# vlongle/pixie

Hardware: AMD Instinct MI355X
Metric: voxels/s (128^3 U-Net fwd) + MPM particle-steps/s (higher is better)
Workload: dtype f32 (operands split fp16 hi+lo, 3 f16 MFMAs/product, fp32 accumulate); 1 GPU; 128^3x64 feature grid -> SegmentationUNet+RegressionUNet forward (+argmax/one-hot combine), 1 scene per GPU per step; grid=128, feature_channels=64, parallelism=scene-parallel x1, executor=c+hip_graph

## Files before the change

pixie_amd/csrc/conv3d_f16x3.hip:

```cpp
#include <hip/hip_runtime.h>

#include <cstdlib>
#include <map>
#include <string>
#include <type_traits>

#include "../../include/pixie_hip.h"
#include "common.h"
#include "conv_plan.h"

namespace pixie {

typedef float f32x16 __attribute__((ext_vector_type(16)));
typedef _Float16 f16x8 __attribute__((ext_vector_type(8)));

constexpr int kW16HeaderU4 = 4;

struct Conv16Args {
    const float* in0; const float* in1;
    int c0, cin;
    int ID, IH, IW;
    int LD, LH, LW;
    int ups;
    int stride;
    int OD, OH, OW;
    const float* pro_a; const float* pro_b; const float* gamma; const float* beta;
    int act;
    const uint4* w16;
    const float* wf;
    const float* bias;
    int cout, coutp;
    const float* residual; float* out;
    const unsigned* amax0; const unsigned* amax1;
    float in_bound;
    int TX, TY, TZ, lTX, lTY;
    int tiles_x, tiles_y, tiles_z, n_tiles;
    int HX, HY, HZ, HYX, CS;
    unsigned mHX, mHYX;
    float* stats; unsigned* out_amax;
    float* partial; int chunks_per_slice;
    int epi_lds;
    const float* sk_in0; const float* sk_in1;
    int sk_c0, sk_cin;
    const uint4* sk_w16; const float* sk_bias;
    const unsigned* sk_amax0; const unsigned* sk_amax1;
};

__device__ __forceinline__ int fast_div16(int n, int d, unsigned magic) {
    return (d == 1) ? n : (int)__umulhi((unsigned)n, magic);
}
__device__ __forceinline__ float act16(float t, int act) {
    if (act == 1) return t > 0.0f ? t : 0.02f * t;
    if (act == 2) return t / (1.0f + __expf(-t));
    return t;
}
__device__ __forceinline__ float act16_staged(float t, int act) {
    if (act == 1) return fmaxf(t, 0.02f * t);
    if (act == 2) return t / (1.0f + __expf(-t));
    return t;
}
__device__ __forceinline__ int scale_exponent(float bound) {
    const unsigned bits = __float_as_uint(bound);
    const int eb = (int)((bits >> 23) & 0xffu) - 127;
    if (!(bound > 0.0f) || eb > 100) return 0;
    int e = 14 - eb;
    return e > 100 ? 100 : (e < -100 ? -100 : e);
}
__device__ __forceinline__ float pow2i(int e) { return __uint_as_float((unsigned)(e + 127) << 23); }

template <int KS, int MB, int NB, bool EX = false, bool SP = false, int SK = 0>
__device__ __forceinline__ void conv3d_f16x3_body(const Conv16Args& A) {
    static_assert(!SP || (KS == 3 && NB == 4 && !EX), "sub-pixel path: 3^3, two x parities x two voxel blocks per wave");
    static_assert(SK == 0 || (!EX && !SP), "folded skip (SK: 1 register-fed, 2 staged through LDS): f16x3, no sub-pixel form");
    extern __shared__ uint4 smem16[];
    constexpr int PAD = (KS == 3) ? 1 : 0;
    constexpr int NW = 4, NT = 64 * NW;
    const int bufsz = 4 * A.CS;

    const int tid = threadIdx.x;
    const int lane = tid & 63;
    const int wave = tid >> 6;
    const int kh = lane >> 5;
    const int l31 = lane & 31;

    int t = blockIdx.x;
    {
        const int per = (A.n_tiles + 7) >> 3;
        const int cand = (t & 7) * per + (t >> 3);
        if ((A.n_tiles & 7) == 0) t = cand;
    }
    int par = 0;
    if constexpr (SP) { par = t & 3; t >>= 2; }
    const int py = par & 1, pz = par >> 1;
    const int tx = t % A.tiles_x; t /= A.tiles_x;
    const int ty = t % A.tiles_y;
    const int tz = t / A.tiles_y;
    const int ox0 = tx * A.TX, oy0 = ty * A.TY, oz0 = tz * A.TZ;
    const int cout0 = blockIdx.y * (MB * 32);
    const int lx0 = SP ? ox0 - 1 : ox0 * A.stride - PAD;
    const int ly0 = SP ? oy0 - 1 + py : oy0 * A.stride - PAD;
    const int lz0 = SP ? oz0 - 1 + pz : oz0 * A.stride - PAD;
    const size_t ISP = (size_t)A.ID * A.IH * A.IW;
    const size_t OSP = (size_t)A.OD * A.OH * A.OW;

    int voff[NB];
    int ovox[NB];
    bool valid[NB];
#pragma unroll
    for (int nb = 0; nb < NB; ++nb) {
        if constexpr (SP) {
            const int px = nb >> 1;
            const int j = (wave * 2 + (nb & 1)) * 32 + l31;
            int x = j & (A.TX - 1);
            int y = (j >> A.lTX) & (A.TY - 1);
            int z = j >> (A.lTX + A.lTY);
            const int gx = 2 * (ox0 + x) + px, gy = 2 * (oy0 + y) + py, gz = 2 * (oz0 + z) + pz;
            const bool v = (z < A.TZ) && (gx < A.OW) && (gy < A.OH) && (gz < A.OD);
            if (!v) { x = 0; y = 0; z = 0; }
            voff[nb] = (z * A.HY + y) * A.HX + x + px + kh * A.CS;
            ovox[nb] = v ? (gz * A.OH + gy) * A.OW + gx : 0;
            valid[nb] = v;
            continue;
        }
        const int j = (wave * NB + nb) * 32 + l31;
        int x = j & (A.TX - 1);
        int y = (j >> A.lTX) & (A.TY - 1);
        int z = j >> (A.lTX + A.lTY);
        const bool v = (z < A.TZ) && (ox0 + x < A.OW) && (oy0 + y < A.OH) && (oz0 + z < A.OD);
        if (!v) { x = 0; y = 0; z = 0; }
        voff[nb] = ((z * A.HY + y) * A.HX + x) * A.stride + kh * A.CS;
        ovox[nb] = ((oz0 + z) * A.OH + (oy0 + y)) * A.OW + ox0 + x;
        valid[nb] = v;
    }

    float bound = A.in_bound;
    if (A.amax0) {
        bound = __uint_as_float(*A.amax0);
        if (A.amax1) bound = fmaxf(bound, __uint_as_float(*A.amax1));
    }
    const int ex = EX ? 0 : scale_exponent(bound);
    const float sx = pow2i(ex);

    f32x16 acc[MB][NB];
#pragma unroll
    for (int mb = 0; mb < MB; ++mb)
#pragma unroll
        for (int nb = 0; nb < NB; ++nb)
#pragma unroll
            for (int r = 0; r < 16; ++r) acc[mb][nb][r] = 0.0f;

    const int KG = A.cin >> 3;
    const size_t tap_stride = (size_t)KG * A.coutp;
    const size_t plane = (size_t)(SP ? 64 : KS * KS * KS) * tap_stride;
    const uint4* wHi = A.w16 + kW16HeaderU4 + (size_t)kh * A.coutp + cout0 + l31 + (size_t)(par * 16) * tap_stride;
    const uint4* wLo = wHi + plane;
    const float* wF = A.wf + (size_t)kh * A.coutp + cout0 + l31;

    constexpr int TAPS = KS * KS * KS;
    auto stage_chunk = [&](int c_base, uint4* buf, int stid, int nthr) {
        uint4* bHi = buf;
        uint4* bLo = buf + 2 * A.CS;
        float pa[16], pb[16];
        {
            float pv = 0.0f;
            if (A.pro_a) pv = (lane & 16) ? A.pro_b[c_base + (lane & 15)] : A.pro_a[c_base + (lane & 15)];
#pragma unroll
            for (int j = 0; j < 16; ++j) {
                pa[j] = __int_as_float(__builtin_amdgcn_readlane(__float_as_int(pv), j));
                pb[j] = __int_as_float(__builtin_amdgcn_readlane(__float_as_int(pv), 16 + j));
            }
        }
        const bool has_aff = A.gamma != nullptr;
        using T = std::true_type; using F = std::false_type;
        if constexpr (EX) {
            float* bF = reinterpret_cast<float*>(buf);
            for (int v0 = stid; v0 < A.CS; v0 += 2 * nthr) {
                float val[2][16];
                float gm[2], bt[2];
                int sidx[2];
                bool ok[2];
#pragma unroll
                for (int u = 0; u < 2; ++u) {
                    const int vox = v0 + u * nthr;
                    int rem = vox;
                    const int hz = fast_div16(rem, A.HYX, A.mHYX);
                    rem -= hz * A.HYX;
                    const int hy = fast_div16(rem, A.HX, A.mHX);
                    const int hx = rem - hy * A.HX;
                    const int lz = lz0 + hz, ly = ly0 + hy, lx = lx0 + hx;
                    ok[u] = vox < A.CS && (unsigned)lz < (unsigned)A.LD && (unsigned)ly < (unsigned)A.LH && (unsigned)lx < (unsigned)A.LW;
                    sidx[u] = ok[u] ? ((lz >> A.ups) * A.IH + (ly >> A.ups)) * A.IW + (lx >> A.ups) : 0;
                }
#pragma unroll
                for (int u = 0; u < 2; ++u) {
#pragma unroll
                    for (int j = 0; j < 16; ++j) {
                        const int cg = c_base + j;
                        const float* src = (cg < A.c0) ? (A.in0 + (size_t)cg * ISP) : (A.in1 + (size_t)(cg - A.c0) * ISP);
                        val[u][j] = src[sidx[u]];
                    }
                    gm[u] = 1.0f; bt[u] = 0.0f;
                    if (has_aff) { gm[u] = A.gamma[sidx[u]]; bt[u] = A.beta[sidx[u]]; }
                }
                auto convert = [&](auto has_pro, auto act_c) {
#pragma unroll
                    for (int u = 0; u < 2; ++u) {
                        const int vox = v0 + u * nthr;
#pragma unroll
                        for (int j = 0; j < 16; ++j) {
                            float t = val[u][j];
                            if (decltype(has_pro)::value) t = t * pa[j] + pb[j];
                            t = t * gm[u] + bt[u];
                            const float sc = ok[u] ? act16(t, decltype(act_c)::value) : 0.0f;
                            if (vox < A.CS) bF[j * A.CS + vox] = sc;
                        }
                    }
                };
                if (A.pro_a) {
                    if (A.act == 1) convert(T{}, std::integral_constant<int, 1>{});
                    else if (A.act == 2) convert(T{}, std::integral_constant<int, 2>{});
                    else convert(T{}, std::integral_constant<int, 0>{});
                } else {
                    if (A.act == 1) convert(F{}, std::integral_constant<int, 1>{});
                    else if (A.act == 2) convert(F{}, std::integral_constant<int, 2>{});
                    else convert(F{}, std::integral_constant<int, 0>{});
                }
            }
            return;
        }
        const int n_items = (A.CS + nthr - 1) / nthr;
        const float* gsrc = has_aff ? A.gamma : A.in0;
        const float* bsrc = has_aff ? A.beta : A.in0;
        constexpr bool BUF = KS == 3 && MB == 2 && NB >= 2 && !SP;
        const unsigned chb = 4u * (unsigned)ISP;
        const int j1 = A.c0 - c_base;
        const bool straddle = j1 > 0 && j1 < 16;
        const float* cbase = (j1 > 0) ? A.in0 + (size_t)c_base * ISP : A.in1 + (size_t)(c_base - A.c0) * ISP;
        const __amdgpu_buffer_rsrc_t rs = __builtin_amdgcn_make_buffer_rsrc(const_cast<float*>(cbase), 0, -1, 0x00020000);
        const __amdgpu_buffer_rsrc_t rsg = __builtin_amdgcn_make_buffer_rsrc(const_cast<float*>(gsrc), 0, -1, 0x00020000);
        const __amdgpu_buffer_rsrc_t rsb = __builtin_amdgcn_make_buffer_rsrc(const_cast<float*>(bsrc), 0, -1, 0x00020000);
        struct Item { float val[16]; float gm, bt; bool ok; };
        auto slot = [&](int vox, bool& ok) {
            int rem = vox;
            const int hz = fast_div16(rem, A.HYX, A.mHYX);
            rem -= hz * A.HYX;
            const int hy = fast_div16(rem, A.HX, A.mHX);
            const int hx = rem - hy * A.HX;
            const int lz = lz0 + hz, ly = ly0 + hy, lx = lx0 + hx;
            ok = vox < A.CS && (unsigned)lz < (unsigned)A.LD && (unsigned)ly < (unsigned)A.LH && (unsigned)lx < (unsigned)A.LW;
            return ok ? ((lz >> A.ups) * A.IH + (ly >> A.ups)) * A.IW + (lx >> A.ups) : 0;
        };
        auto load_with_pointers = [&](Item& it, int sidx) {
            it.gm = gsrc[sidx]; it.bt = bsrc[sidx];
#pragma unroll
            for (int j = 0; j < 16; ++j) {
                const int cg = c_base + j;
                const float* src = (cg < A.c0) ? (A.in0 + (size_t)cg * ISP) : (A.in1 + (size_t)(cg - A.c0) * ISP);
                it.val[j] = src[sidx];
            }
        };
        auto fetch = [&](Item& it, int vox) {
            const int sidx = slot(vox, it.ok);
            if constexpr (BUF) {
                const int voff = 4 * sidx;
                it.gm = __uint_as_float(__builtin_amdgcn_raw_buffer_load_b32(rsg, voff, 0, 0));
                it.bt = __uint_as_float(__builtin_amdgcn_raw_buffer_load_b32(rsb, voff, 0, 0));
#pragma unroll
                for (int j = 0; j < 16; ++j)
                    it.val[j] = __uint_as_float(__builtin_amdgcn_raw_buffer_load_b32(rs, voff, (int)((unsigned)j * chb), 0));
            } else {
                load_with_pointers(it, sidx);
            }
            __builtin_amdgcn_sched_barrier(0);
        };
        auto convert = [&](const Item& it, int vox, auto has_pro, auto act_c) {
            const float gm = has_aff ? it.gm : 1.0f, bt = has_aff ? it.bt : 0.0f;
            f16x8 vh[2], vl[2];
#pragma unroll
            for (int j = 0; j < 16; ++j) {
                float t = it.val[j];
                if (decltype(has_pro)::value) t = t * pa[j] + pb[j];
                t = t * gm + bt;
                const float sc = act16_staged(t, decltype(act_c)::value) * sx;
                const _Float16 h = (_Float16)sc;
                vh[j >> 3][j & 7] = h;
                vl[j >> 3][j & 7] = (_Float16)(sc - (float)h);
            }
            uint4 w[4] = {__builtin_bit_cast(uint4, vh[0]), __builtin_bit_cast(uint4, vh[1]), __builtin_bit_cast(uint4, vl[0]),
                          __builtin_bit_cast(uint4, vl[1])};
#pragma unroll
            for (int q = 0; q < 4; ++q) {
                w[q].x = it.ok ? w[q].x : 0u; w[q].y = it.ok ? w[q].y : 0u;
                w[q].z = it.ok ? w[q].z : 0u; w[q].w = it.ok ? w[q].w : 0u;
            }
            if (vox < A.CS) {
                bHi[vox] = w[0];
                bHi[A.CS + vox] = w[1];
                bLo[vox] = w[2];
                bLo[A.CS + vox] = w[3];
            }
            __builtin_amdgcn_sched_barrier(0);
        };
        auto pipeline = [&](auto has_pro, auto act_c) {
            Item a, b;
            int vox = stid;
            int left = n_items;
            if constexpr (BUF) {
                if (straddle) {
#pragma unroll 1
                    for (; left > 0; --left, vox += nthr) {
                        load_with_pointers(a, slot(vox, a.ok));
                        convert(a, vox, has_pro, act_c);
                    }
                    return;
                }
            }
            fetch(a, vox);
#pragma unroll 1
            for (; left > 2; left -= 2, vox += 2 * nthr) {
                fetch(b, vox + nthr);
                convert(a, vox, has_pro, act_c);
                fetch(a, vox + 2 * nthr);
                convert(b, vox + nthr, has_pro, act_c);
            }
            if (left == 2) {
                fetch(b, vox + nthr);
                convert(a, vox, has_pro, act_c);
                convert(b, vox + nthr, has_pro, act_c);
            } else {
                convert(a, vox, has_pro, act_c);
            }
        };
        if (A.pro_a) {
            if (A.act == 1) pipeline(T{}, std::integral_constant<int, 1>{});
            else if (A.act == 2) pipeline(T{}, std::integral_constant<int, 2>{});
            else pipeline(T{}, std::integral_constant<int, 0>{});
        } else {
            if (A.act == 1) pipeline(F{}, std::integral_constant<int, 1>{});
            else if (A.act == 2) pipeline(F{}, std::integral_constant<int, 2>{});
            else pipeline(F{}, std::integral_constant<int, 0>{});
        }
    };
    auto mfma_chunk = [&](int c_base, const uint4* buf) {
        __builtin_amdgcn_s_setprio(3);
        if constexpr (EX) {
            const float* ldsF = reinterpret_cast<const float*>(buf);
            const size_t tapw = (size_t)A.cin * A.coutp;
            const float* wc = wF + (size_t)c_base * A.coutp;
            float a[8][MB], an[8][MB];
#pragma unroll
            for (int kp = 0; kp < 8; ++kp)
#pragma unroll
                for (int mb = 0; mb < MB; ++mb) a[kp][mb] = wc[(size_t)(2 * kp) * A.coutp + mb * 32];
#pragma unroll 1
            for (int zy = 0; zy < KS * KS; ++zy) {
                const int dz = zy / KS, dy = zy - dz * KS;
                const int rowoff = (dz * A.HY + dy) * A.HX;
#pragma unroll
// ... 82 lines not shown
        f16x8 ah[MB], al[MB];
#pragma unroll
        for (int mb = 0; mb < MB; ++mb) {
            ah[mb] = __builtin_bit_cast(f16x8, wh[mb * 32]);
            al[mb] = __builtin_bit_cast(f16x8, wl[mb * 32]);
        }
#pragma unroll 1
        for (int zy = 0; zy < KS * KS; ++zy) {
            const int dz = zy / KS, dy = zy - dz * KS;
            const int rowoff = (dz * A.HY + dy) * A.HX;
#pragma unroll
            for (int dx = 0; dx < KS; ++dx) {
                const int tap = zy * KS + dx;
                const int nxt = (tap + 1 < TAPS) ? tap + 1 : tap;
                f16x8 ahn[MB], aln[MB];
#pragma unroll
                for (int mb = 0; mb < MB; ++mb) {
                    ahn[mb] = __builtin_bit_cast(f16x8, wh[(size_t)nxt * tap_stride + mb * 32]);
                    aln[mb] = __builtin_bit_cast(f16x8, wl[(size_t)nxt * tap_stride + mb * 32]);
                }
                __builtin_amdgcn_sched_barrier(0);
                f16x8 bh[NB], bl[NB];
#pragma unroll
                for (int nb = 0; nb < NB; ++nb) {
                    bh[nb] = __builtin_bit_cast(f16x8, ldsHi[voff[nb] + rowoff + dx]);
                    bl[nb] = __builtin_bit_cast(f16x8, ldsLo[voff[nb] + rowoff + dx]);
                }
#pragma unroll
                for (int mb = 0; mb < MB; ++mb)
#pragma unroll
                    for (int nb = 0; nb < NB; ++nb)
                        acc[mb][nb] = __builtin_amdgcn_mfma_f32_32x32x16_f16(al[mb], bh[nb], acc[mb][nb], 0, 0, 0);
#pragma unroll
                for (int mb = 0; mb < MB; ++mb)
#pragma unroll
                    for (int nb = 0; nb < NB; ++nb)
                        acc[mb][nb] = __builtin_amdgcn_mfma_f32_32x32x16_f16(ah[mb], bl[nb], acc[mb][nb], 0, 0, 0);
#pragma unroll
                for (int mb = 0; mb < MB; ++mb)
#pragma unroll
                    for (int nb = 0; nb < NB; ++nb)
                        acc[mb][nb] = __builtin_amdgcn_mfma_f32_32x32x16_f16(ah[mb], bh[nb], acc[mb][nb], 0, 0, 0);
#pragma unroll
                for (int mb = 0; mb < MB; ++mb) { ah[mb] = ahn[mb]; al[mb] = aln[mb]; }
            }
        }
        __builtin_amdgcn_s_setprio(0);
    };

    float inv2 = 0.0f;
    {
        const int c_begin = A.partial ? (int)blockIdx.z * A.chunks_per_slice * 16 : 0;
        const int c_end = A.partial ? min(A.cin, c_begin + A.chunks_per_slice * 16) : A.cin;
        for (int c_base = c_begin; c_base < c_end; c_base += 16) {
            __syncthreads();
            stage_chunk(c_base, smem16, tid, NT);
            __syncthreads();
            mfma_chunk(c_base, smem16);
        }
        if constexpr (SK != 0) {
            float sb = __uint_as_float(*A.sk_amax0);
            if (A.sk_amax1) sb = fmaxf(sb, __uint_as_float(*A.sk_amax1));
            const int ex2 = scale_exponent(sb);
            const float sx2 = pow2i(ex2);
            const float inv_main = __uint_as_float(A.w16[0].x) * pow2i(-ex);
            inv2 = __uint_as_float(A.sk_w16[0].x) * pow2i(-ex2);
            const float ratio = inv_main / inv2;
#pragma unroll
            for (int mb = 0; mb < MB; ++mb)
#pragma unroll
                for (int nb = 0; nb < NB; ++nb)
#pragma unroll
                    for (int r = 0; r < 16; ++r) acc[mb][nb][r] *= ratio;
            auto sk_chunks = [&]() {
                int l31s = l31, khs = kh, waves = wave;
                asm volatile("" : "+v"(l31s), "+v"(khs), "+v"(waves));
                const unsigned chb = 4u * (unsigned)ISP;
                unsigned off[NB];
#pragma unroll
                for (int nb = 0; nb < NB; ++nb) {
                    const int j = (waves * NB + nb) * 32 + l31s;
                    const int x = j & (A.TX - 1), y = (j >> A.lTX) & (A.TY - 1), z = j >> (A.lTX + A.lTY);
                    off[nb] = (valid[nb] ? 4u * (unsigned)(((oz0 + z) * A.IH + (oy0 + y)) * A.IW + ox0 + x) : 0u) + 8u * (unsigned)khs * chb;
                }
                const unsigned wlane = 16u * (unsigned)(khs * A.coutp + l31s);
                const char* w2Hi = reinterpret_cast<const char*>(A.sk_w16 + kW16HeaderU4 + cout0);
                const char* w2Lo = w2Hi + (size_t)(A.sk_cin >> 3) * A.coutp * sizeof(uint4);
#pragma unroll 1
                for (int c2 = 0; c2 < A.sk_cin; c2 += 16) {
                    f16x8 ah[MB], al[MB];
                    const size_t wrow = (size_t)(c2 >> 3) * A.coutp * sizeof(uint4);
#pragma unroll
                    for (int mb = 0; mb < MB; ++mb) {
                        al[mb] = __builtin_bit_cast(f16x8, *reinterpret_cast<const uint4*>(w2Lo + wrow + mb * 32 * sizeof(uint4) + wlane));
                        ah[mb] = __builtin_bit_cast(f16x8, *reinterpret_cast<const uint4*>(w2Hi + wrow + mb * 32 * sizeof(uint4) + wlane));
                    }
                    const float* base = (c2 < A.sk_c0) ? (A.sk_in0 + (size_t)c2 * ISP) : (A.sk_in1 + (size_t)(c2 - A.sk_c0) * ISP);
                    const __amdgpu_buffer_rsrc_t rsrc = __builtin_amdgcn_make_buffer_rsrc(const_cast<float*>(base), 0, -1, 0x00020000);
                    float v[NB][8];
#pragma unroll
                    for (int q = 0; q < 8; ++q)
#pragma unroll
                        for (int nb = 0; nb < NB; ++nb)
                            v[nb][q] = __uint_as_float(__builtin_amdgcn_raw_buffer_load_b32(rsrc, (int)off[nb], (int)((unsigned)q * chb), 0));
                    __builtin_amdgcn_sched_barrier(0);
                    f16x8 bh[NB], bl[NB];
#pragma unroll
                    for (int nb = 0; nb < NB; ++nb)
#pragma unroll
                        for (int q = 0; q < 8; ++q) {
                            const float sc = valid[nb] ? v[nb][q] * sx2 : 0.0f;
// ... 55 lines not shown
                            vl[q >> 3][q & 7] = (_Float16)(sc - (float)hq);
                        }
                        const int slot = (z * A.HY + y) * A.HX + x + centre;
                        bHi[slot] = __builtin_bit_cast(uint4, vh[0]);
                        bHi[A.CS + slot] = __builtin_bit_cast(uint4, vh[1]);
                        bLo[slot] = __builtin_bit_cast(uint4, vl[0]);
                        bLo[A.CS + slot] = __builtin_bit_cast(uint4, vl[1]);
                    }
                    __syncthreads();
                    f16x8 bh[NB], bl[NB];
#pragma unroll
                    for (int nb = 0; nb < NB; ++nb) {
                        bh[nb] = __builtin_bit_cast(f16x8, bHi[voff[nb] + centre]);
                        bl[nb] = __builtin_bit_cast(f16x8, bLo[voff[nb] + centre]);
                    }
#pragma unroll
                    for (int mb = 0; mb < MB; ++mb)
#pragma unroll
                        for (int nb = 0; nb < NB; ++nb)
                            acc[mb][nb] = __builtin_amdgcn_mfma_f32_32x32x16_f16(al[mb], bh[nb], acc[mb][nb], 0, 0, 0);
#pragma unroll
                    for (int mb = 0; mb < MB; ++mb)
#pragma unroll
                        for (int nb = 0; nb < NB; ++nb)
                            acc[mb][nb] = __builtin_amdgcn_mfma_f32_32x32x16_f16(ah[mb], bl[nb], acc[mb][nb], 0, 0, 0);
#pragma unroll
                    for (int mb = 0; mb < MB; ++mb)
#pragma unroll
                        for (int nb = 0; nb < NB; ++nb)
                            acc[mb][nb] = __builtin_amdgcn_mfma_f32_32x32x16_f16(ah[mb], bh[nb], acc[mb][nb], 0, 0, 0);
                }
            } else {
                sk_chunks();
            }
        }
    }

    const float inv = EX ? 1.0f : (SK != 0 ? inv2 : __uint_as_float(A.w16[0].x) * pow2i(-ex));
    if (A.partial) {
        float* dst = A.partial + (size_t)blockIdx.z * A.cout * OSP;
#pragma unroll
        for (int mb = 0; mb < MB; ++mb)
#pragma unroll
            for (int r = 0; r < 16; ++r) {
                const int co = cout0 + mb * 32 + (r & 3) + 8 * (r >> 2) + 4 * kh;
                if (co < A.cout) {
#pragma unroll
                    for (int nb = 0; nb < NB; ++nb)
                        if (valid[nb]) dst[(size_t)co * OSP + ovox[nb]] = acc[mb][nb][r] * inv;
                }
            }
        return;
    }
    float* red = reinterpret_cast<float*>(smem16);
    float wmax = 0.0f;
    const bool full = SP ? (A.epi_lds && cout0 + MB * 32 <= A.cout && (A.TX & 1) == 0 && (A.OW & 3) == 0 && NW * 64 <= A.TX * A.TY * A.TZ &&
                            2 * (ox0 + A.TX) <= A.OW && 2 * (oy0 + A.TY) <= A.OH && 2 * (oz0 + A.TZ) <= A.OD)
                         : (A.epi_lds && cout0 + MB * 32 <= A.cout && (A.TX & 3) == 0 && (A.OW & 3) == 0 && NW * NB * 32 <= A.TX * A.TY * A.TZ &&
                            ox0 + A.TX <= A.OW && oy0 + A.TY <= A.OH && oz0 + A.TZ <= A.OD);
    if (full) {
        constexpr int LDO = NB * 32 + 4;
        float* ldsO = reinterpret_cast<float*>(smem16) + wave * (32 * LDO);
        red = reinterpret_cast<float*>(smem16) + NW * 32 * LDO;
        constexpr int LPR = NB * 8;
        constexpr int RPI = 32 / LPR;
        constexpr int NIT = 16 / RPI;
        constexpr int G = 4;
        constexpr int GPB = NIT / G;
        constexpr int NGRP = MB * GPB;
        const int rsub = l31 / LPR, colq = 4 * (l31 % LPR), nbq = colq >> 5;
        const float* nobias = EX ? A.wf : reinterpret_cast<const float*>(A.w16);
        const bool hb0 = A.bias != nullptr, hb1 = A.sk_bias != nullptr;
        float braw[MB][2];
#pragma unroll
        for (int mb = 0; mb < MB; ++mb) {
            braw[mb][0] = (hb0 ? A.bias : nobias)[cout0 + mb * 32 + l31];
            braw[mb][1] = (hb1 ? A.sk_bias : nobias)[cout0 + mb * 32 + l31];
        }
        __syncthreads();
        const int jq = SP ? wave * 64 + (colq >> 1) : (wave * NB + nbq) * 32 + (colq & 31);
        const int xq = jq & (A.TX - 1), yq = (jq >> A.lTX) & (A.TY - 1), zq = jq >> (A.lTX + A.lTY);
        const size_t ovq = SP ? ((size_t)(2 * (oz0 + zq) + pz) * A.OH + (2 * (oy0 + yq) + py)) * A.OW + 2 * (ox0 + xq)
                              : ((size_t)(oz0 + zq) * A.OH + (oy0 + yq)) * A.OW + ox0 + xq;
        const size_t orow0 = (size_t)(cout0 + kh * RPI + rsub) * OSP + ovq;
        auto rows = [&](auto res_c, auto stats_c) {
            constexpr bool RES = decltype(res_c)::value, STATS = decltype(stats_c)::value;
            size_t step = (size_t)(2 * RPI) * OSP;
            asm volatile("" : "+s"(step));
            const float* pr = A.residual + orow0;
            float* po = A.out + orow0;
            float4 r4[2][G];
            auto fetch = [&](int q) {
#pragma unroll
                for (int g = 0; g < G; ++g) { r4[q & 1][g] = *reinterpret_cast<const float4*>(pr); pr += step; }
            };
#pragma unroll
            for (int q = 0; q < NGRP; ++q) {
                const int mb = q / GPB, it0 = (q % GPB) * G;
                asm volatile("" ::: "memory");
                if (q % GPB == 0) {
                    const int brow = __float_as_int((hb0 ? braw[mb][0] : 0.0f) + (hb1 ? braw[mb][1] : 0.0f));
#pragma unroll
                    for (int r = 0; r < 16; ++r) {
                        const int row = (r & 3) + 8 * (r >> 2);
                        const int blo = __builtin_amdgcn_readlane(brow, row), bhi = __builtin_amdgcn_readlane(brow, row + 4);
                        const float bv = __int_as_float(kh ? bhi : blo);
#pragma unroll
                        for (int nb = 0; nb < NB; ++nb)
                            ldsO[((r & 3) + 8 * (r >> 2) + 4 * kh) * LDO + (SP ? 2 * ((nb & 1) * 32 + l31) + (nb >> 1) : nb * 32 + l31)] =
                                __builtin_fmaf(acc[mb][nb][r], inv, bv);
                    }
                }
                if constexpr (RES) {
                    if (q == 0) fetch(0);
                    if (q + 1 < NGRP) fetch(q + 1);
                }
                float4 v4[G];
#pragma unroll
                for (int g = 0; g < G; ++g) {
                    const int rowl = (2 * (it0 + g) + kh) * RPI + rsub;
                    v4[g] = *reinterpret_cast<const float4*>(ldsO + rowl * LDO + colq);
                    if constexpr (RES) { v4[g].x += r4[q & 1][g].x; v4[g].y += r4[q & 1][g].y; v4[g].z += r4[q & 1][g].z; v4[g].w += r4[q & 1][g].w; }
                    *reinterpret_cast<float4*>(po) = v4[g]; po += step;
                }
                if constexpr (STATS) {
                    float s1[G], s2[G];
#pragma unroll
                    for (int g = 0; g < G; ++g) {
                        const float4 v = v4[g];
                        s1[g] = (v.x + v.y) + (v.z + v.w);
                        s2[g] = (v.x * v.x + v.y * v.y) + (v.z * v.z + v.w * v.w);
                        wmax = fmaxf(fmaxf(wmax, fmaxf(fabsf(v.x), fabsf(v.y))), fmaxf(fabsf(v.z), fabsf(v.w)));
                    }
                    asm volatile("" : "+v"(wmax));
#pragma unroll
                    for (int off = LPR / 2; off > 0; off >>= 1) {
                        float t1[G], t2[G];
#pragma unroll
                        for (int g = 0; g < G; ++g) { t1[g] = __shfl_xor(s1[g], off, 64); t2[g] = __shfl_xor(s2[g], off, 64); }
#pragma unroll
                        for (int g = 0; g < G; ++g) { s1[g] += t1[g]; s2[g] += t2[g]; }
                    }
                    if ((l31 % LPR) == 0) {
#pragma unroll
                        for (int g = 0; g < G; ++g) {
                            const int rowl = (2 * (it0 + g) + kh) * RPI + rsub;
                            red[(wave * MB * 32 + mb * 32 + rowl) * 2] = s1[g]; red[(wave * MB * 32 + mb * 32 + rowl) * 2 + 1] = s2[g];
                        }
                    }
                }
            }
        };
        using T = std::true_type; using F = std::false_type;
        if (A.residual) { if (A.stats) rows(T{}, T{}); else rows(T{}, F{}); }
        else { if (A.stats) rows(F{}, T{}); else rows(F{}, F{}); }
    } else {
    if (A.stats) __syncthreads();
#pragma unroll
    for (int mb = 0; mb < MB; ++mb) {
#pragma unroll
        for (int r = 0; r < 16; ++r) {
            const int row = mb * 32 + (r & 3) + 8 * (r >> 2) + 4 * kh;
            const int co = cout0 + row;
            float s1 = 0.0f, s2 = 0.0f;
            if (co < A.cout) {
                const float bv = (A.bias ? A.bias[co] : 0.0f) + (A.sk_bias ? A.sk_bias[co] : 0.0f);
#pragma unroll
                for (int nb = 0; nb < NB; ++nb) {
                    if (valid[nb]) {
                        const size_t o = (size_t)co * OSP + ovox[nb];
                        float val = acc[mb][nb][r] * inv + bv;
                        if (A.residual) val += A.residual[o];
                        A.out[o] = val;
                        s1 += val; s2 += val * val; wmax = fmaxf(wmax, fabsf(val));
                    }
                }
            }
            if (A.stats) {
#pragma unroll
                for (int off = 16; off > 0; off >>= 1) { s1 += __shfl_xor(s1, off, 64); s2 += __shfl_xor(s2, off, 64); }
                if (l31 == 0) { red[(wave * MB * 32 + row) * 2] = s1; red[(wave * MB * 32 + row) * 2 + 1] = s2; }
            }
        }
    }
    }
    if (A.stats) {
        __syncthreads();
        if (tid < MB * 32 * 2) {
            float t = red[tid];
#pragma unroll
            for (int w = 1; w < NW; ++w) t += red[w * MB * 64 + tid];
            A.stats[((size_t)blockIdx.x * A.coutp + cout0) * 2 + tid] = t;
        }
        if (A.out_amax) {
#pragma unroll
            for (int off = 32; off > 0; off >>= 1) wmax = fmaxf(wmax, __shfl_xor(wmax, off, 64));
            if (lane == 0 && wmax > 0.0f) atomicMax(A.out_amax, __float_as_uint(wmax));
        }
    }
}

template <int KS, int MB, int NB>
__global__ __launch_bounds__(256, 2) void conv3d_f16x3_kernel(Conv16Args A) {
    conv3d_f16x3_body<KS, MB, NB>(A);
}
template <int KS, int MB, int NB, bool STAGED>
__global__ __launch_bounds__(256, 2) void conv3d_f16x3_skip_kernel(Conv16Args A) {
    conv3d_f16x3_body<KS, MB, NB, false, false, STAGED ? 2 : 1>(A);
}
template <int KS, int MB, int NB>
__global__ __launch_bounds__(256, 2) void conv3d_exact_kernel(Conv16Args A) {
    conv3d_f16x3_body<KS, MB, NB, true>(A);
}
template <int MB>
__global__ __launch_bounds__(256, 2) void conv3d_f16x3_subpixel_kernel(Conv16Args A) {
    conv3d_f16x3_body<3, MB, 4, false, true>(A);
}
__global__ __launch_bounds__(256, 2) void conv3d_f16x3_c64_fullres_kernel(Conv16Args A) {
    conv3d_f16x3_body<3, 2, 4>(A);
}

struct StatParts { const void* p; int n; long cstride, tstride; int f64; };

__device__ inline void block_channel_sums(const StatParts& P, int c, double* r, double& o1, double& o2) {
    double s1 = 0.0, s2 = 0.0;
    for (int t = threadIdx.x; t < P.n; t += 256) {
        const size_t k = ((size_t)c * P.cstride + (size_t)t * P.tstride) * 2;
        if (P.f64) { const double2 v = *reinterpret_cast<const double2*>(static_cast<const double*>(P.p) + k); s1 += v.x; s2 += v.y; }
        else { const float2 v = *reinterpret_cast<const float2*>(static_cast<const float*>(P.p) + k); s1 += v.x; s2 += v.y; }
    }
    for (int off = 32; off > 0; off >>= 1) { s1 += __shfl_down(s1, off, 64); s2 += __shfl_down(s2, off, 64); }
    if ((threadIdx.x & 63) == 0) { r[2 * (threadIdx.x >> 6)] = s1; r[2 * (threadIdx.x >> 6) + 1] = s2; }
    __syncthreads();
    o1 = r[0] + r[2] + r[4] + r[6]; o2 = r[1] + r[3] + r[5] + r[7];
    __syncthreads();
}

__global__ __launch_bounds__(256) void stats_finalize_kernel(StatParts P, double* __restrict__ sums) {
    const int c = blockIdx.x;
    __shared__ double r[8];
    double s1, s2;
    block_channel_sums(P, c, r, s1, s2);
    if (threadIdx.x == 0) { sums[2 * c] = s1; sums[2 * c + 1] = s2; }
}

__global__ __launch_bounds__(256) void stats_norm_finalize_kernel(StatParts P0, double* sums0, int c0, StatParts P1, double* sums1, int channels,
                                                                  double spatial, int mode, int groups, double eps,
                                                                  const float* __restrict__ weight, const float* __restrict__ bias,
                                                                  float* __restrict__ a, float* __restrict__ b) {
    __shared__ double r[8];
    const int cpg = mode == 0 ? 1 : channels / groups;
    const int first = blockIdx.x * cpg;
    double s1 = 0.0, s2 = 0.0;
    for (int k = first; k < first + cpg; ++k) {
        const bool in0 = k < c0;
        const StatParts& P = in0 ? P0 : P1;
        double* sums = in0 ? sums0 : sums1;
// ... 275 lines not shown
            for (int nb = NB; nb >= 1 && !found; nb /= 2) {
                for (int sl = 1; sl <= smax; sl *= 2)
                    if (n_wg(MB, nb) * sl >= 512) { NB = nb; slices = sl; found = true; break; }
            }
            if (!found) { NB = 1; slices = 1; while (slices * 2 <= smax) slices *= 2; }
        } else {
            while (n_wg(MB, NB) < 512 && NB > 1) NB /= 2;
            if (n_wg(MB, NB) < 512 && MB > 1) MB = 1;
        }
        p.MB = MB; p.NB = NB; p.slices = slices;
        tile(p.OD, p.OH, p.OW, 128 * NB);
        p.HX = (p.TX - 1) * s.stride + s.ksize; p.HY = (p.TY - 1) * s.stride + s.ksize; p.HZ = (p.TZ - 1) * s.stride + s.ksize;
    }
    p.HYX = p.HY * p.HX; p.CS = p.HZ * p.HYX;
    p.mHX = magic_of(p.HX); p.mHYX = magic_of(p.HYX);
    if (p.slices > 1) p.chunks_per_slice = (chunks + p.slices - 1) / p.slices;
    p.lds_bytes = (size_t)4 * p.CS * sizeof(uint4);
    if (p.lds_bytes > 160 * 1024) return refuse(CONV_BAD_LDS);
    const size_t epi_bytes = ((size_t)4 * 32 * (p.NB * 32 + 4) + (size_t)4 * p.MB * 32 * 2) * sizeof(float);
    if (p.slices == 1 && epi_bytes <= 80 * 1024) { p.epi_lds = 1; p.lds_bytes = std::max(p.lds_bytes, epi_bytes); }
    p.grid = dim3((unsigned)p.n_tiles, (unsigned)((p.coutp + p.MB * 32 - 1) / (p.MB * 32)), (unsigned)p.slices);
    if (!p.f16x3()) return p;
    const long osp = (long)p.OD * p.OH * p.OW;
    if (p.slices > 1) {
        const int n = reduce_segments(osp);
        p.stats = ConvStatLayout{n, n, 1, 1};
        p.stats_floats = (int64_t)s.c_out * n * 2 * (int64_t)(sizeof(double) / sizeof(float));
        p.workspace_bytes = (int64_t)p.slices * s.c_out * osp * (int64_t)sizeof(float);
    } else {
        p.stats = ConvStatLayout{p.n_tiles, 1, p.coutp, 0};
        p.stats_floats = (int64_t)p.n_tiles * p.coutp * 2;
    }
    p.fullres = !sub && p.slices == 1 && s.ksize == 3 && p.MB == 2 && p.NB == 4 && cin == 64 && s.c_out == 64 && s.stride == 1 && !s.upsample &&
                s.c1 == 0 && !s.skip && osp >= 128L * 128 * 128;
    const int scin = s.skip_c0 + s.skip_c1;
    p.skip_foldable = !sub && s.stride == 1 && !s.upsample && scin > 0 && scin % 16 == 0 && s.skip_c0 % 8 == 0 && p.slices == 1;
    return p;
}

using ConvKernel = void (*)(Conv16Args);
static ConvKernel conv16_kernel(const ConvPlan& p, bool skip = false, int skip_c0 = 0) {
    if (p.path == CONV_F16X3_SUBPIXEL) return p.MB == 2 ? conv3d_f16x3_subpixel_kernel<2> : conv3d_f16x3_subpixel_kernel<1>;
    if (p.fullres) return conv3d_f16x3_c64_fullres_kernel;
#define PX_CONV16_PICK(KS_, MB_, NB_)                                                                \
    if (p.KS == KS_ && p.MB == MB_ && p.NB == NB_)                                                   \
        return p.path == CONV_EXACT_TILED ? conv3d_exact_kernel<KS_, MB_, NB_>                       \
                                          : (!skip ? conv3d_f16x3_kernel<KS_, MB_, NB_>                                \
                                                   : ((skip_c0 & 8) ? conv3d_f16x3_skip_kernel<KS_, MB_, NB_, true> : conv3d_f16x3_skip_kernel<KS_, MB_, NB_, false>));
    PX_CONV_VARIANTS(PX_CONV16_PICK)
#undef PX_CONV16_PICK
    return nullptr;
}

static int launch(ConvKernel kern, const ConvPlan& p, const Conv16Args& a, hipStream_t st) {
    PX_REQUIRE(kern != nullptr, "conv: no kernel variant for ksize=%d MB=%d NB=%d", p.KS, p.MB, p.NB);
    PX_CHECK_HIP(allow_max_dynamic_lds(reinterpret_cast<const void*>(kern)));
    hipLaunchKernelGGL(kern, p.grid, dim3(256), p.lds_bytes, st, a);
    PX_CHECK_HIP(hipGetLastError());
    return 0;
}

static Conv16Args conv16_args(const pixie_conv_desc* d, const ConvPlan& p) {
    Conv16Args a{};
    a.in0 = d->d_in0; a.in1 = d->d_in1; a.c0 = d->c0; a.cin = d->c0 + d->c1;
    a.ID = d->in_d; a.IH = d->in_h; a.IW = d->in_w;
    a.LD = p.LD; a.LH = p.LH; a.LW = p.LW; a.ups = p.ups; a.stride = d->stride;
    a.OD = p.OD; a.OH = p.OH; a.OW = p.OW;
    a.pro_a = d->d_pro_a; a.pro_b = d->d_pro_b; a.gamma = d->d_gamma; a.beta = d->d_beta; a.act = d->act;
    a.bias = d->d_bias; a.cout = d->c_out; a.coutp = p.coutp;
    a.residual = d->d_residual; a.out = d->d_out;
    a.TX = p.TX; a.TY = p.TY; a.TZ = p.TZ; a.lTX = p.lTX; a.lTY = p.lTY;
    a.tiles_x = p.tiles_x; a.tiles_y = p.tiles_y; a.tiles_z = p.tiles_z; a.n_tiles = p.n_tiles;
    a.HX = p.HX; a.HY = p.HY; a.HZ = p.HZ; a.HYX = p.HYX; a.CS = p.CS; a.mHX = p.mHX; a.mHYX = p.mHYX;
    a.chunks_per_slice = p.chunks_per_slice; a.epi_lds = p.epi_lds;
    return a;
}

int conv3d_f16x3_forward(const pixie_conv_desc* d, const ConvPlan& p, hipStream_t st) {
    PX_REQUIRE(p.refusal != CONV_BAD_STRIDE, "f16x3 conv: stride must be 1, or 2 for a 3^3 kernel");
    PX_REQUIRE(p.refusal != CONV_BAD_CHANNELS, "f16x3 conv: c_in must be a multiple of 16 (got %d+%d)", d->c0, d->c1);
    PX_REQUIRE(d->d_in_amax0 != nullptr || d->in_bound > 0.0f, "f16x3 conv: needs d_in_amax0 or a positive in_bound");
    PX_REQUIRE(d->c1 == 0 || d->d_in_amax0 == nullptr || d->d_in_amax1 != nullptr, "f16x3 conv: second input needs its own amax slot");
    PX_REQUIRE(p.refusal != CONV_BAD_SUBPIXEL, "f16x3 conv: sub-pixel weights need upsample = 1, ksize = 3, stride = 1 and no folded skip");
    PX_REQUIRE((int64_t)d->in_d * d->in_h * d->in_w * 16 * (int64_t)sizeof(float) < (int64_t)1 << 32, "f16x3 conv: 16 channels of the input must span less than 4 GiB");
    Conv16Args a = conv16_args(d, p);
    a.w16 = reinterpret_cast<const uint4*>(d->d_w16);
    a.amax0 = d->d_in_amax0; a.amax1 = (d->c1 > 0) ? d->d_in_amax1 : nullptr; a.in_bound = d->in_bound;
    a.stats = d->d_out_stats; a.out_amax = d->d_out_amax;
    if (d->d_skip_w16) {
        PX_REQUIRE(p.skip_foldable, "f16x3 conv: this launch cannot fold a skip convolution (pixie_conv_skip_foldable)");
        PX_REQUIRE(d->d_skip_in0 && d->d_skip_amax0 && (d->skip_c1 == 0 || (d->d_skip_in1 && d->d_skip_amax1)), "f16x3 conv: folded skip needs its inputs and their amax slots");
        PX_REQUIRE((int64_t)d->in_d * d->in_h * d->in_w * 16 * (int64_t)sizeof(float) < (int64_t)1 << 32, "f16x3 conv: folded skip: 16 channels of the skip input must span less than 4 GiB");
        a.sk_in0 = d->d_skip_in0; a.sk_in1 = d->d_skip_in1; a.sk_c0 = d->skip_c0; a.sk_cin = d->skip_c0 + d->skip_c1;
        a.sk_w16 = reinterpret_cast<const uint4*>(d->d_skip_w16); a.sk_bias = d->d_skip_bias;
        a.sk_amax0 = d->d_skip_amax0; a.sk_amax1 = d->skip_c1 > 0 ? d->d_skip_amax1 : nullptr;
    }
    if (p.slices > 1) {
        a.partial = static_cast<float*>(d->d_workspace);
        a.stats = nullptr; a.out_amax = nullptr;
    }
    PX_REQUIRE(p.refusal != CONV_BAD_LDS, "f16x3 conv: tile needs %zu B of LDS", p.lds_bytes);
    PX_REQUIRE(p.f16x3(), "f16x3 conv: bad sizes");
    if (int rc = launch(conv16_kernel(p, a.sk_w16 != nullptr, a.sk_c0), p, a, st)) return rc;
    if (p.slices == 1) return 0;
    const long osp = (long)a.OD * a.OH * a.OW, n_elems = (long)a.cout * osp;
    if (d->d_out_stats) {
        const dim3 rgrid((unsigned)reduce_segments(osp), (unsigned)a.cout);
        double* rstats = reinterpret_cast<double*>(d->d_out_stats);
        PX_REQUIRE((reinterpret_cast<size_t>(rstats) & 7) == 0, "f16x3 conv: d_out_stats of a split-K launch must be 8-byte aligned");
        const bool vec = osp % 4 == 0 && ((reinterpret_cast<size_t>(a.partial) | reinterpret_cast<size_t>(a.residual) | reinterpret_cast<size_t>(a.out)) & 15) == 0;
        if (vec) hipLaunchKernelGGL(splitk_reduce_stats_kernel<true>, rgrid, dim3(256), 0, st, a.partial, p.slices, n_elems, osp, a.bias, a.residual,
                                    a.out, rstats, d->d_out_amax);
        else hipLaunchKernelGGL(splitk_reduce_stats_kernel<false>, rgrid, dim3(256), 0, st, a.partial, p.slices, n_elems, osp, a.bias, a.residual,
                                a.out, rstats, d->d_out_amax);
    } else {
        hipLaunchKernelGGL(splitk_reduce_kernel, dim3((unsigned)((n_elems + 255) / 256)), dim3(256), 0, st, a.partial, p.slices, n_elems, osp,
                           a.bias, a.residual, a.out);
    }
    PX_CHECK_HIP(hipGetLastError());
    return 0;
}

int conv3d_exact_forward(const pixie_conv_desc* d, const ConvPlan& p, hipStream_t st) {
    PX_REQUIRE(p.refusal != CONV_BAD_LDS, "exact conv: tile needs %zu B of LDS", p.lds_bytes);
    PX_REQUIRE(p.path == CONV_EXACT_TILED, "exact conv: bad sizes");
    Conv16Args a = conv16_args(d, p);
    a.wf = d->d_w;
    a.in_bound = 1.0f;
    return launch(conv16_kernel(p), p, a, st);
}

}

using namespace pixie;

static ConvPlan plan_of(const pixie_conv_desc* d) { return d ? conv_plan(conv_shape_of(d)) : ConvPlan{}; }
static StatParts stat_parts(const ConvPlan& p, const void* stats) { return StatParts{stats, p.stats.n, p.stats.cstride, p.stats.tstride, p.stats.f64}; }

extern "C" int64_t pixie_conv_stats_floats(const pixie_conv_desc* d) { return plan_of(d).stats_floats; }

extern "C" int64_t pixie_conv_workspace_bytes(const pixie_conv_desc* d) {
    if (!d) return 0;
    ConvShape s = conv_shape_of(d);
    s.workspace = true;
    return conv_plan(s).workspace_bytes;
}

#ifdef PIXIE_DIAG
extern "C" int pixie_conv_kernel_variant(const pixie_conv_desc* d, int* slices_out) {
    const ConvPlan p = plan_of(d);
    if (slices_out) *slices_out = p.f16x3() ? p.slices : 1;
    if (!p.f16x3()) return 0;
    if (p.path == CONV_F16X3_SUBPIXEL) return 8300 + p.MB * 10 + p.NB;
    if (p.fullres) return 9324;
    return p.KS * 100 + p.MB * 10 + p.NB;
}

extern "C" int pixie_conv_tile_geometry(const pixie_conv_desc* d, int32_t out[10]) {
    const ConvPlan p = plan_of(d);
    if (!out || !p.tiled()) return 1;
    const int32_t v[10] = {p.TX, p.TY, p.TZ, p.tiles_x, p.tiles_y, p.tiles_z, p.epi_lds, p.slices, p.MB, p.NB};
    for (int i = 0; i < 10; ++i) out[i] = v[i];
    return 0;
}

extern "C" int pixie_conv_stats_layout(const pixie_conv_desc* d, int64_t out[6]) {
    const ConvPlan p = plan_of(d);
    if (!out || !p.f16x3()) return 1;
    out[0] = p.stats.n; out[1] = p.stats.cstride; out[2] = p.stats.tstride; out[3] = p.stats.f64; out[4] = p.stats.f64 ? kReduceSeg : 0;
    out[5] = p.coutp;
    return 0;
}
#endif

extern "C" int pixie_conv_skip_foldable(const pixie_conv_desc* d) { return plan_of(d).skip_foldable ? 1 : 0; }

extern "C" int pixie_stats_finalize(const float* d_stats, const pixie_conv_desc* d, double* d_sums, void* stream) {
    PX_REQUIRE(d_stats && d && d_sums, "pixie_stats_finalize: null argument");
    hipLaunchKernelGGL(stats_finalize_kernel, dim3((unsigned)d->c_out), dim3(256), 0, as_stream(stream), stat_parts(plan_of(d), d_stats), d_sums);
    PX_CHECK_HIP(hipGetLastError());
    return 0;
}

extern "C" int pixie_stats_norm_finalize(const float* d_stats0, const pixie_conv_desc* desc0, double* d_sums0, const float* d_stats1,
                                         const pixie_conv_desc* desc1, double* d_sums1, int c1, int64_t spatial, int mode, int groups,
                                         double eps, const float* d_weight, const float* d_bias, float* d_a, float* d_b, void* stream) {
    PX_REQUIRE(desc0 && d_sums0 && d_a && d_b && spatial > 0 && c1 >= 0, "pixie_stats_norm_finalize: bad arguments");
    PX_REQUIRE(c1 == 0 || d_sums1, "pixie_stats_norm_finalize: a second part needs d_sums1");
    PX_REQUIRE(!d_stats1 || desc1, "pixie_stats_norm_finalize: d_stats1 needs its descriptor");
    const int c0 = desc0->c_out, channels = c0 + c1;
    PX_REQUIRE(!d_stats1 || desc1->c_out == c1, "pixie_stats_norm_finalize: desc1 has %d output channels, c1 is %d", desc1 ? desc1->c_out : 0, c1);
    PX_REQUIRE(mode == 0 || (mode == 1 && groups > 0 && channels % groups == 0), "pixie_stats_norm_finalize: bad mode/groups");
    const StatParts none{nullptr, 0, 0, 0, 0};
    const StatParts p0 = d_stats0 ? stat_parts(plan_of(desc0), d_stats0) : none;
    const StatParts p1 = d_stats1 ? stat_parts(plan_of(desc1), d_stats1) : none;
    hipLaunchKernelGGL(stats_norm_finalize_kernel, dim3((unsigned)(mode == 0 ? channels : groups)), dim3(256), 0, as_stream(stream), p0, d_sums0, c0,
                       p1, d_sums1, channels, (double)spatial, mode, groups, eps, d_weight, d_bias, d_a, d_b);
    PX_CHECK_HIP(hipGetLastError());
    return 0;
}

extern "C" int64_t pixie_conv_packed16_bytes(int c_out, int c_in, int ksize) {
    if (c_out <= 0 || c_in <= 0 || c_in % 8 != 0 || (ksize != 1 && ksize != 3)) return 0;
    const int64_t taps = (int64_t)ksize * ksize * ksize;
    return ((int64_t)kW16HeaderU4 + 2 * taps * (c_in / 8) * pixie_conv_cout_padded(c_out)) * (int64_t)sizeof(uint4);
}

extern "C" int pixie_tensor_amax(const float* d_x, int64_t count, uint32_t* d_slot, void* stream) {
    PX_REQUIRE(d_x && d_slot && count > 0, "pixie_tensor_amax: bad arguments");
    const int blocks = (int)std::min<int64_t>(2048, (count + 1023) / 1024);
    hipLaunchKernelGGL(amax_kernel, dim3(blocks), dim3(256), 0, as_stream(stream), d_x, (long)count, d_slot);
    PX_CHECK_HIP(hipGetLastError());
// ... 41 lines not shown
```

Baseline: 26.55 million voxels/s.

## Pair two four-wave quartets per block to share staging and overlap MFMA

Adds a 512-thread pair variant of the f16x3 conv kernel where two quartets of waves cover adjacent 64-channel c_out blocks for the same voxel tile. Each quartet stages half of the shared input tile into double-buffered LDS, and staging of the next chunk alternates with MFMA on the current chunk across the quartets. This halves per-block input staging work and overlaps loads with matrix math, at the cost of larger LDS use, one block per CU, and reduced grid.y. It is used only for eligible non-skip, non-split-K MB=2 NB=4 plans with coutp divisible by 128.

```diff
diff --git a/pixie_amd/csrc/conv3d_f16x3.hip b/pixie_amd/csrc/conv3d_f16x3.hip
--- a/pixie_amd/csrc/conv3d_f16x3.hip
+++ b/pixie_amd/csrc/conv3d_f16x3.hip
@@ -68,8 +68,9 @@
 }
 __device__ __forceinline__ float pow2i(int e) { return __uint_as_float((unsigned)(e + 127) << 23); }
 
-template <int KS, int MB, int NB, bool EX = false, bool SP = false, int SK = 0>
+template <int KS, int MB, int NB, bool EX = false, bool SP = false, int SK = 0, bool PAIR = false>
 __device__ __forceinline__ void conv3d_f16x3_body(const Conv16Args& A) {
+    static_assert(!PAIR || (MB == 2 && !EX && !SP && SK == 0), "pair form: the plain f16x3 body with 64 c_out per quartet");
     static_assert(!SP || (KS == 3 && NB == 4 && !EX), "sub-pixel path: 3^3, two x parities x two voxel blocks per wave");
     static_assert(SK == 0 || (!EX && !SP), "folded skip (SK: 1 register-fed, 2 staged through LDS): f16x3, no sub-pixel form");
     extern __shared__ uint4 smem16[];
@@ -79,7 +80,9 @@
 
     const int tid = threadIdx.x;
     const int lane = tid & 63;
-    const int wave = tid >> 6;
+    const int quartet = PAIR ? __builtin_amdgcn_readfirstlane(tid >> 8) : 0;
+    const int wave = PAIR ? (tid >> 6) & 3 : tid >> 6;
+    const int qtid = PAIR ? tid & 255 : tid;
     const int kh = lane >> 5;
     const int l31 = lane & 31;
 
@@ -96,7 +99,7 @@
     const int ty = t % A.tiles_y;
     const int tz = t / A.tiles_y;
     const int ox0 = tx * A.TX, oy0 = ty * A.TY, oz0 = tz * A.TZ;
-    const int cout0 = blockIdx.y * (MB * 32);
+    const int cout0 = (PAIR ? 2 * (int)blockIdx.y + quartet : (int)blockIdx.y) * (MB * 32);
     const int lx0 = SP ? ox0 - 1 : ox0 * A.stride - PAD;
     const int ly0 = SP ? oy0 - 1 + py : oy0 * A.stride - PAD;
     const int lz0 = SP ? oz0 - 1 + pz : oz0 * A.stride - PAD;
@@ -157,7 +160,7 @@
     const float* wF = A.wf + (size_t)kh * A.coutp + cout0 + l31;
 
     constexpr int TAPS = KS * KS * KS;
-    auto stage_chunk = [&](int c_base, uint4* buf, int stid, int nthr) {
+    auto stage_chunk = [&](int c_base, uint4* buf, int stid, int nthr, int s0, int s1) {
         uint4* bHi = buf;
         uint4* bLo = buf + 2 * A.CS;
         float pa[16], pb[16];
@@ -228,7 +231,7 @@
             }
             return;
         }
-        const int n_items = (A.CS + nthr - 1) / nthr;
+        const int n_items = (s1 - s0 + nthr - 1) / nthr;
         const float* gsrc = has_aff ? A.gamma : A.in0;
         const float* bsrc = has_aff ? A.beta : A.in0;
         constexpr bool BUF = KS == 3 && MB == 2 && NB >= 2 && !SP;
@@ -247,7 +250,7 @@
             const int hy = fast_div16(rem, A.HX, A.mHX);
             const int hx = rem - hy * A.HX;
             const int lz = lz0 + hz, ly = ly0 + hy, lx = lx0 + hx;
-            ok = vox < A.CS && (unsigned)lz < (unsigned)A.LD && (unsigned)ly < (unsigned)A.LH && (unsigned)lx < (unsigned)A.LW;
+            ok = vox < s1 && (unsigned)lz < (unsigned)A.LD && (unsigned)ly < (unsigned)A.LH && (unsigned)lx < (unsigned)A.LW;
             return ok ? ((lz >> A.ups) * A.IH + (ly >> A.ups)) * A.IW + (lx >> A.ups) : 0;
         };
         auto load_with_pointers = [&](Item& it, int sidx) {
@@ -293,7 +296,7 @@
                 w[q].x = it.ok ? w[q].x : 0u; w[q].y = it.ok ? w[q].y : 0u;
                 w[q].z = it.ok ? w[q].z : 0u; w[q].w = it.ok ? w[q].w : 0u;
             }
-            if (vox < A.CS) {
+            if (vox < s1) {
                 bHi[vox] = w[0];
                 bHi[A.CS + vox] = w[1];
                 bLo[vox] = w[2];
@@ -303,7 +306,7 @@
         };
         auto pipeline = [&](auto has_pro, auto act_c) {
             Item a, b;
-            int vox = stid;
+            int vox = s0 + stid;
             int left = n_items;
             if constexpr (BUF) {
                 if (straddle) {
@@ -492,11 +495,26 @@
     {
         const int c_begin = A.partial ? (int)blockIdx.z * A.chunks_per_slice * 16 : 0;
         const int c_end = A.partial ? min(A.cin, c_begin + A.chunks_per_slice * 16) : A.cin;
+        if constexpr (PAIR) {
+            const int n_chunks = (c_end - c_begin) >> 4;
+            const int half = (A.CS + 1) >> 1;
+            const int s0 = quartet ? half : 0, s1 = quartet ? A.CS : half;
+#pragma unroll 1
+            for (int h = -1; h < 2 * n_chunks; ++h) {
+                const int k = h >> 1;
+                const bool stage = (h < 0 || ((h + quartet) & 1) == 0) && k + 1 < n_chunks;
+                const bool multiply = h >= 0 && ((h + quartet) & 1) != 0;
+                if (stage) stage_chunk(c_begin + 16 * (k + 1), smem16 + ((k + 1) & 1) * bufsz, qtid, NT, s0, s1);
+                if (multiply) mfma_chunk(c_begin + 16 * k, smem16 + (k & 1) * bufsz);
+                if (h & 1) __syncthreads();
+            }
+        } else {
         for (int c_base = c_begin; c_base < c_end; c_base += 16) {
             __syncthreads();
-            stage_chunk(c_base, smem16, tid, NT);
+            stage_chunk(c_base, smem16, tid, NT, 0, A.CS);
             __syncthreads();
             mfma_chunk(c_base, smem16);
+        }
         }
         if constexpr (SK != 0) {
             float sb = __uint_as_float(*A.sk_amax0);
@@ -658,7 +676,8 @@
             }
         return;
     }
-    float* red = reinterpret_cast<float*>(smem16);
+    constexpr int LDO_ = NB * 32 + 4;
+    float* red = reinterpret_cast<float*>(smem16) + (PAIR ? (A.epi_lds ? 2 * NW * 32 * LDO_ : 0) + quartet * (NW * MB * 64) : 0);
     float wmax = 0.0f;
     const bool full = SP ? (A.epi_lds && cout0 + MB * 32 <= A.cout && (A.TX & 1) == 0 && (A.OW & 3) == 0 && NW * 64 <= A.TX * A.TY * A.TZ &&
                             2 * (ox0 + A.TX) <= A.OW && 2 * (oy0 + A.TY) <= A.OH && 2 * (oz0 + A.TZ) <= A.OD)
@@ -666,8 +685,8 @@
                             ox0 + A.TX <= A.OW && oy0 + A.TY <= A.OH && oz0 + A.TZ <= A.OD);
     if (full) {
         constexpr int LDO = NB * 32 + 4;
-        float* ldsO = reinterpret_cast<float*>(smem16) + wave * (32 * LDO);
-        red = reinterpret_cast<float*>(smem16) + NW * 32 * LDO;
+        float* ldsO = reinterpret_cast<float*>(smem16) + (quartet * NW + wave) * (32 * LDO);
+        if constexpr (!PAIR) red = reinterpret_cast<float*>(smem16) + NW * 32 * LDO;
         constexpr int LPR = NB * 8;
         constexpr int RPI = 32 / LPR;
         constexpr int NIT = 16 / RPI;
@@ -761,7 +780,7 @@
         if (A.residual) { if (A.stats) rows(T{}, T{}); else rows(T{}, F{}); }
         else { if (A.stats) rows(F{}, T{}); else rows(F{}, F{}); }
     } else {
-    if (A.stats) __syncthreads();
+    if (PAIR || A.stats) __syncthreads();
 #pragma unroll
     for (int mb = 0; mb < MB; ++mb) {
 #pragma unroll
@@ -792,11 +811,11 @@
     }
     if (A.stats) {
         __syncthreads();
-        if (tid < MB * 32 * 2) {
-            float t = red[tid];
-#pragma unroll
-            for (int w = 1; w < NW; ++w) t += red[w * MB * 64 + tid];
-            A.stats[((size_t)blockIdx.x * A.coutp + cout0) * 2 + tid] = t;
+        if (qtid < MB * 32 * 2) {
+            float t = red[qtid];
+#pragma unroll
+            for (int w = 1; w < NW; ++w) t += red[w * MB * 64 + qtid];
+            A.stats[((size_t)blockIdx.x * A.coutp + cout0) * 2 + qtid] = t;
         }
         if (A.out_amax) {
 #pragma unroll
@@ -809,6 +828,10 @@
 template <int KS, int MB, int NB>
 __global__ __launch_bounds__(256, 2) void conv3d_f16x3_kernel(Conv16Args A) {
     conv3d_f16x3_body<KS, MB, NB>(A);
+}
+template <int KS, int NB>
+__global__ __launch_bounds__(512, 1) void conv3d_f16x3_pair_kernel(Conv16Args A) {
+    conv3d_f16x3_body<KS, 2, NB, false, false, 0, true>(A);
 }
 template <int KS, int MB, int NB, bool STAGED>
 __global__ __launch_bounds__(256, 2) void conv3d_f16x3_skip_kernel(Conv16Args A) {
@@ -1190,10 +1213,33 @@
     return nullptr;
 }
 
-static int launch(ConvKernel kern, const ConvPlan& p, const Conv16Args& a, hipStream_t st) {
+#ifdef PIXIE_DIAG
+static int g_conv_keep_four_wave = 0;
+#endif
+static size_t conv_pair_lds(const ConvPlan& p, bool skip) {
+#ifdef PIXIE_DIAG
+    if (g_conv_keep_four_wave) return 0;
+#endif
+    if (p.path != CONV_F16X3 || p.fullres || skip || p.MB != 2 || p.NB != 4 || p.slices != 1 || p.coutp % 128 != 0) return 0;
+    const size_t tiles = (size_t)2 * 4 * p.CS * sizeof(uint4);
+    const size_t red = (size_t)2 * 4 * p.MB * 32 * 2 * sizeof(float);
+    const size_t epi = p.epi_lds ? (size_t)8 * 32 * (p.NB * 32 + 4) * sizeof(float) + red : red;
+    const size_t lds = std::max(tiles, epi);
+    return lds <= 160 * 1024 ? lds : 0;
+}
+static ConvKernel conv16_pair_kernel(const ConvPlan& p) {
+#define PX_CONV16_PAIR(KS_, NB_) \
+    if (p.KS == KS_ && p.NB == NB_) return conv3d_f16x3_pair_kernel<KS_, NB_>;
+    PX_CONV16_PAIR(3, 4) PX_CONV16_PAIR(1, 4)
+#undef PX_CONV16_PAIR
+    return nullptr;
+}
+
+static int launch(ConvKernel kern, const ConvPlan& p, const Conv16Args& a, hipStream_t st, size_t pair_lds = 0) {
     PX_REQUIRE(kern != nullptr, "conv: no kernel variant for ksize=%d MB=%d NB=%d", p.KS, p.MB, p.NB);
     PX_CHECK_HIP(allow_max_dynamic_lds(reinterpret_cast<const void*>(kern)));
-    hipLaunchKernelGGL(kern, p.grid, dim3(256), p.lds_bytes, st, a);
+    if (pair_lds) hipLaunchKernelGGL(kern, dim3(p.grid.x, p.grid.y / 2, 1), dim3(512), pair_lds, st, a);
+    else hipLaunchKernelGGL(kern, p.grid, dim3(256), p.lds_bytes, st, a);
     PX_CHECK_HIP(hipGetLastError());
     return 0;
 }
@@ -1239,7 +1285,8 @@
     }
     PX_REQUIRE(p.refusal != CONV_BAD_LDS, "f16x3 conv: tile needs %zu B of LDS", p.lds_bytes);
     PX_REQUIRE(p.f16x3(), "f16x3 conv: bad sizes");
-    if (int rc = launch(conv16_kernel(p, a.sk_w16 != nullptr, a.sk_c0), p, a, st)) return rc;
+    const size_t pair_lds = conv_pair_lds(p, a.sk_w16 != nullptr);
+    if (int rc = launch(pair_lds ? conv16_pair_kernel(p) : conv16_kernel(p, a.sk_w16 != nullptr, a.sk_c0), p, a, st, pair_lds)) return rc;
     if (p.slices == 1) return 0;
     const long osp = (long)a.OD * a.OH * a.OW, n_elems = (long)a.cout * osp;
     if (d->d_out_stats) {
@@ -1286,6 +1333,11 @@
 
 #ifdef PIXIE_DIAG
 extern "C" int pixie_conv_kernel_variant(const pixie_conv_desc* d, int* slices_out) {
+    if (!d) {
+        const int before = g_conv_keep_four_wave;
+        if (slices_out && (*slices_out == 0 || *slices_out == 1)) g_conv_keep_four_wave = *slices_out;
+        return before;
+    }
     const ConvPlan p = plan_of(d);
     if (slices_out) *slices_out = p.f16x3() ? p.slices : 1;
     if (!p.f16x3()) return 0;
@@ -1296,6 +1348,7 @@
 
 extern "C" int pixie_conv_tile_geometry(const pixie_conv_desc* d, int32_t out[10]) {
     const ConvPlan p = plan_of(d);
+    if (!out && d) return (int)conv_pair_lds(p, d->d_skip_w16 != nullptr);
     if (!out || !p.tiled()) return 1;
     const int32_t v[10] = {p.TX, p.TY, p.TZ, p.tiles_x, p.tiles_y, p.tiles_z, p.epi_lds, p.slices, p.MB, p.NB};
     for (int i = 0; i < 10; ++i) out[i] = v[i];
```

Result: faster. 26.88 million voxels/s (median of 6 runs) (+1.2%).
